# ignacio-rocco/detectorch

Measured on AMD Instinct MI355X. Metric: images/sec Mask R-CNN R-50-FPN 1333x800 (region-proposal hot path), higher is better.
Workload: dtype f32

## Files before the change

### detectorch_amd/csrc/roi_align_tile.hip

```cpp

#include <type_traits>

#include "roi_align_common.h"

namespace dtc {

constexpr int kTileMaxK = 32;
constexpr int kTileRoiBytes = 48, kTileGroupBytes = 32;
constexpr int kTileHdrBytes = kTileMaxK * (kTileRoiBytes + kTileGroupBytes) + 16;
template <int NT> struct TileShape;
template <> struct TileShape<256> { static constexpr int kUnits = 8, kWaves = 3, kLdsKB = 52, kWaves16 = 4, kLds16KB = 38; };

struct TileRoi {
  int lvl, b, x0, x1, y0, y1, r, valid;
  float sh, sw, bin_h, bin_w;
};
static_assert(sizeof(TileRoi) == kTileRoiBytes, "TileRoi layout");
struct TileGroup { int first, count, kind, x0, x1, y0, y1, pad; };
enum { kGrpPool = 0, kGrpZero = 1, kGrpAbsent = 2, kGrpGather = 3 };

__device__ __forceinline__ __amdgpu_buffer_rsrc_t make_srd(const void* base) {
  return __builtin_amdgcn_make_buffer_rsrc(const_cast<void*>(base), 0, 0xffffffff, 0x00020000);
}
template <typename TIn> struct Piece4;
template <> struct Piece4<float> {
  typedef float4 Raw;
  static __device__ __forceinline__ Raw raw(__amdgpu_buffer_rsrc_t r, uint32_t voff, uint32_t soff) {
    const u32x4 v = __builtin_amdgcn_raw_buffer_load_b128(r, voff, soff, 0);
    return make_float4(__uint_as_float(v.x), __uint_as_float(v.y), __uint_as_float(v.z), __uint_as_float(v.w));
  }
};
template <> struct Piece4<__half> {
  typedef u32x2 Raw;
  static __device__ __forceinline__ Raw raw(__amdgpu_buffer_rsrc_t r, uint32_t voff, uint32_t soff) { return __builtin_amdgcn_raw_buffer_load_b64(r, voff, soff, 0); }
};
template <> struct Piece4<bf16_t> {
  typedef u32x2 Raw;
  static __device__ __forceinline__ Raw raw(__amdgpu_buffer_rsrc_t r, uint32_t voff, uint32_t soff) { return __builtin_amdgcn_raw_buffer_load_b64(r, voff, soff, 0); }
};

template <typename TIn> struct TileLds { typedef float T; static constexpr int kSlot = 16, kShift = 4; };
template <> struct TileLds<__half> { typedef uint16_t T; static constexpr int kSlot = 8, kShift = 3; };
template <> struct TileLds<bf16_t> { typedef uint16_t T; static constexpr int kSlot = 8, kShift = 3; };

template <typename TIn, int NT> struct TileBounds { static constexpr int kWaves = TileShape<NT>::kWaves; };
template <int NT> struct TileBounds<__half, NT> { static constexpr int kWaves = TileShape<NT>::kWaves16; };
template <int NT> struct TileBounds<bf16_t, NT> { static constexpr int kWaves = TileShape<NT>::kWaves16; };

__device__ __forceinline__ int tile_phys(int px) { return px + (px >> 3); }

struct TileItem {
  int a[2][2][4];
  float yl[2], yh[2], xl[2], xh[2];
  bool on;
};

enum { kStageScalar = 0, kStageVec = 1, kStageVecUnaligned = 2 };

struct TileGeom {
  int first, count;
  int y0, x0a, ngx, npos;
  int plane;
  int nq_pass;
  int mode;
};

template <typename TIn, typename TOut, int NT, bool FUSED>
__device__ __forceinline__ void tile_passes(const RoiAlignParams& p, const dtc_feat_level& L, const TIn* fbase, int c0, int nc,
                                            int bins, float* slab, typename TileLds<TIn>::T* win, const TileRoi* troi, const TileGeom& g,
                                            const TileItem& it, int rl, int bin) {
  constexpr int NW = NT / 64;
  constexpr int U = TileShape<NT>::kUnits;
  typedef typename TileLds<TIn>::T TL;
  constexpr bool L16 = sizeof(TL) == 2;
  constexpr int SB = TileLds<TIn>::kSlot;
  const int tid = threadIdx.x, lane = tid & 63, wv = tid >> 6, pl = lane & 15, cl = (lane >> 4) & 3;
  const int npos = g.npos, ngx = g.ngx, plane = g.plane, nq_pass = g.nq_pass;
  const int nchunk = (npos + 15) >> 4;
  const int KC = ceil_div(nchunk, NW);
  const float rinv = 1.0f / (float)ngx;
  const int nq_tot = ceil_div(nc, 4);
  const bool vec = g.mode != kStageScalar;
  uint32_t uoff[U];
  int ulds[U];
  const int nu = KC * nq_pass;
  if (vec) {
    const int sh32 = (int)L.stride_h, sc32 = (int)L.stride_c;
    int q = 0, i = 0;
#pragma unroll
    for (int u = 0; u < U; u++) {
      const bool dup = u >= nu;
      const int pos = min((wv + (dup ? 0 : i) * NW) * 16 + pl, npos - 1);
      const int row = (int)(((float)pos + 0.5f) * rinv);
      const int gx = pos - row * ngx;
      const int qq = dup ? 0 : q;
      int col = g.x0a + 4 * gx, sft = 0;
      if (g.mode == kStageVecUnaligned) { sft = max(0, col + 3 - (L.width - 1)); col -= sft; }
      uoff[u] = ((uint32_t)((g.y0 + row) * sh32 + col + (4 * qq + cl) * sc32) * (uint32_t)sizeof(TIn)) | ((uint32_t)sft << 30);
      ulds[u] = qq * plane * 4 + ((4 * pos + (pos >> 1)) << 2) + cl;
      if (++i == KC) { i = 0; q++; }
    }
  }
  const __amdgpu_buffer_rsrc_t srd = make_srd(fbase);
  const uint32_t pass_bytes = (uint32_t)(L.stride_c * (int64_t)sizeof(TIn));
  typename Piece4<TIn>::Raw v[U];
  auto issue = [&](int cs) {
    const uint32_t soff = (uint32_t)cs * pass_bytes;
    if (g.mode == kStageVec) {
#pragma unroll
      for (int u = 0; u < U; u++) v[u] = Piece4<TIn>::raw(srd, uoff[u], soff);
    } else {
#pragma unroll
      for (int u = 0; u < U; u++) v[u] = Piece4<TIn>::raw(srd, uoff[u] & 0x3fffffffu, soff);
    }
  };
  auto commit_as = [&](auto shifted_tag) {
    constexpr bool SHIFTED = decltype(shifted_tag)::value;
    if constexpr (SHIFTED) asm volatile("" ::: "memory");
#pragma unroll
    for (int u = 0; u < U; u++) {
      if constexpr (L16) {
        uint32_t w0 = v[u].x & 0xffffu, w1 = v[u].x >> 16, w2 = v[u].y & 0xffffu, w3 = v[u].y >> 16;
        if constexpr (SHIFTED) {
          const uint32_t sft = uoff[u] >> 30;
          w0 = sft == 0 ? w0 : sft == 1 ? w1 : sft == 2 ? w2 : w3;
          w1 = sft == 0 ? w1 : sft == 1 ? w2 : w3;
          w2 = sft == 0 ? w2 : w3;
        }
        TL* d = win + ulds[u];
        d[0] = (TL)w0; d[4] = (TL)w1; d[8] = (TL)w2; d[12] = (TL)w3;
      } else {
        float4 w = v[u];
        if constexpr (SHIFTED) {
          const uint32_t sft = uoff[u] >> 30;
          w.x = sft == 0 ? w.x : sft == 1 ? w.y : sft == 2 ? w.z : w.w;
          w.y = sft == 0 ? w.y : sft == 1 ? w.z : w.w;
          w.z = sft == 0 ? w.z : w.w;
        }
        TL* d = win + ulds[u];
        d[0] = w.x; d[4] = w.y; d[8] = w.z; d[12] = w.w;
      }
    }
  };
  auto commit = [&]() {
    if (g.mode == kStageVecUnaligned) commit_as(std::true_type{}); else commit_as(std::false_type{});
  };
  auto lds_val = [&](const TIn& x) -> TL {
    if constexpr (L16) return *reinterpret_cast<const uint16_t*>(&x); else return to_f32<TIn>(x);
  };
  auto stage_scalar = [&](int cs) {
#pragma unroll 1
    for (int q = 0; q < nq_pass; q++) {
      const int cq = cs + 4 * q;
      if (cq >= nc) break;
      const int cle = min(cl, nc - 1 - cq);
      const TIn* base = fbase + (int64_t)(cq + cle) * L.stride_c;
#pragma unroll 1
      for (int t = wv; t < nchunk; t += NW) {
        const int pos = min(t * 16 + pl, npos - 1);
        const int row = (int)(((float)pos + 0.5f) * rinv);
        const int gx = pos - row * ngx;
        const int rem = L.width - 1 - (g.x0a + 4 * gx);
        const TIn* s = base + (int64_t)(g.y0 + row) * L.stride_h + (int64_t)(g.x0a + 4 * gx) * L.stride_w;
        TL* d = win + q * plane * 4 + ((4 * pos + (pos >> 1)) << 2) + cl;
        d[0] = lds_val(s[0]);
        d[4] = lds_val(s[(int64_t)min(1, rem) * L.stride_w]);
        d[8] = lds_val(s[(int64_t)min(2, rem) * L.stride_w]);
        d[12] = lds_val(s[(int64_t)min(3, rem) * L.stride_w]);
      }
    }
  };
  const bool quad_ok = ((p.channels | c0) & 3) == 0;
  auto store_slab = [&](int cs, int nq) {
    const int nch = min(4 * nq, nc - cs);
    TOut* out = reinterpret_cast<TOut*>(p.out);
    if (quad_ok && nch == 4 * nq) {
      const int n4 = nq * bins, total = g.count * n4;
      const float r4 = 1.0f / (float)n4;
      const int cs_off = cs * bins;
      for (int idx = tid; idx < total; idx += NT) {
        const int k = (int)(((float)idx + 0.5f) * r4);
        const int e = idx - __mul24(k, n4);
        const float4 val = reinterpret_cast<const float4*>(slab)[idx];
        const uint64_t ob = *reinterpret_cast<const uint64_t*>(&troi[g.first + k].x0);
        store4<TOut>(out + (ob + (uint64_t)(uint32_t)(cs_off + 4 * e)), val);
      }
    } else {
      const int per = nch * bins, total = g.count * per;
      for (int idx = tid; idx < total; idx += NT) {
        const int k = idx / per, e = idx - k * per;
        out[((size_t)troi[g.first + k].r * p.channels + c0 + cs) * bins + e] = from_f32<TOut>(slab[k * 4 * nq * bins + e]);
      }
    }
  };

  if (vec) issue(0);
  int cs_prev = 0, nq_prev = 0;
#pragma unroll 1
  for (int qs = 0; qs < nq_tot; qs += nq_pass) {
    const int cs = 4 * qs;
    const int nq_cur = min(nq_pass, nq_tot - qs);
    if (vec) commit(); else stage_scalar(cs);
    if (nq_prev) store_slab(cs_prev, nq_prev);
    __syncthreads();
    if (vec && qs + nq_pass < nq_tot) issue(cs + 4 * nq_pass);
    if (it.on) {
      float* so = slab + rl * (4 * nq_cur * bins) + bin;
#pragma unroll 1
      for (int q = 0; q < nq_cur; q++) {
        const char* wq = reinterpret_cast<const char*>(win) + uni(q * plane * SB);
        f32x2 a01 = {0.f, 0.f}, a23 = {0.f, 0.f};
#pragma unroll
        for (int iy = 0; iy < 2; iy++) {
          if constexpr (L16 && FUSED) {
            u32x2 t[2][4];
#pragma unroll
            for (int ix = 0; ix < 2; ix++)
#pragma unroll
              for (int k = 0; k < 4; k++)
                t[ix][k] = *reinterpret_cast<const u32x2*>(__builtin_assume_aligned(wq + it.a[iy][ix][k], 8));
#pragma unroll
            for (int ix = 0; ix < 2; ix++) {
              const float w1 = it.yh[iy] * it.xh[ix], w2 = it.yh[iy] * it.xl[ix];
              const float w3 = it.yl[iy] * it.xh[ix], w4 = it.yl[iy] * it.xl[ix];
              fma_pair16<TIn>(a01, t[ix][0].x, w1); fma_pair16<TIn>(a23, t[ix][0].y, w1);
              fma_pair16<TIn>(a01, t[ix][1].x, w2); fma_pair16<TIn>(a23, t[ix][1].y, w2);
              fma_pair16<TIn>(a01, t[ix][2].x, w3); fma_pair16<TIn>(a23, t[ix][2].y, w3);
              fma_pair16<TIn>(a01, t[ix][3].x, w4); fma_pair16<TIn>(a23, t[ix][3].y, w4);
            }
          } else if constexpr (L16) {
            u32x2 t[2][4];
#pragma unroll
            for (int ix = 0; ix < 2; ix++)
#pragma unroll
              for (int k = 0; k < 4; k++)
                t[ix][k] = *reinterpret_cast<const u32x2*>(__builtin_assume_aligned(wq + it.a[iy][ix][k], 8));
#pragma unroll
            for (int ix = 0; ix < 2; ix++) {
              const float w1 = it.yh[iy] * it.xh[ix], w2 = it.yh[iy] * it.xl[ix];
              const float w3 = it.yl[iy] * it.xh[ix], w4 = it.yl[iy] * it.xl[ix];
              f32x2 s01 = mul_pair16<TIn>(t[ix][0].x, w1) + mul_pair16<TIn>(t[ix][1].x, w2);
              s01 = s01 + mul_pair16<TIn>(t[ix][2].x, w3);
              s01 = s01 + mul_pair16<TIn>(t[ix][3].x, w4);
              f32x2 s23 = mul_pair16<TIn>(t[ix][0].y, w1) + mul_pair16<TIn>(t[ix][1].y, w2);
              s23 = s23 + mul_pair16<TIn>(t[ix][2].y, w3);
              s23 = s23 + mul_pair16<TIn>(t[ix][3].y, w4);
              a01 = a01 + s01; a23 = a23 + s23;
            }
          } else {
            f32x4 t[2][4];
#pragma unroll
            for (int ix = 0; ix < 2; ix++)
#pragma unroll
              for (int k = 0; k < 4; k++)
                t[ix][k] = *reinterpret_cast<const f32x4*>(__builtin_assume_aligned(wq + it.a[iy][ix][k], 16));
#pragma unroll
            for (int ix = 0; ix < 2; ix++) {
              const float w1 = it.yh[iy] * it.xh[ix], w2 = it.yh[iy] * it.xl[ix];
              const float w3 = it.yl[iy] * it.xh[ix], w4 = it.yl[iy] * it.xl[ix];
              a01 += w1 * t[ix][0].lo + w2 * t[ix][1].lo + w3 * t[ix][2].lo + w4 * t[ix][3].lo;
              a23 += w1 * t[ix][0].hi + w2 * t[ix][1].hi + w3 * t[ix][2].hi + w4 * t[ix][3].hi;
            }
          }
          __builtin_amdgcn_sched_barrier(0);
        }
        float* o = so + uni(4 * q * bins);
        const float a0 = a01.x, a1 = a01.y, a2 = a23.x, a3 = a23.y;
        o[0] = a0 * 0.25f; o[bins] = a1 * 0.25f; o[2 * bins] = a2 * 0.25f; o[3 * bins] = a3 * 0.25f;
      }
    }
    __syncthreads();
    cs_prev = cs; nq_prev = nq_cur;
  }
  if (nq_prev) store_slab(cs_prev, nq_prev);
}

__device__ __forceinline__ int tile_work_item(int b, int n, int reverse) {
  if (n < 2 * kXcds || (reverse & 2)) return (reverse & 1) ? n - 1 - b : b;
  const int x = b % kXcds, j = b / kXcds;
  const int q = n / kXcds, r = n - q * kXcds;
  const int start = x * q + min(x, r), qx = q + (x < r ? 1 : 0);
  return start + ((reverse & 1) ? qx - 1 - j : j);
}

template <typename TIn, typename TOut, int NT, bool FUSED>
__global__ __launch_bounds__(NT, (TileBounds<TIn, NT>::kWaves)) void roi_align_fwd_tile(RoiAlignParams p, int kgroup, int lds_bytes, int nq_cap, int merge_pct, int reverse) {
  extern __shared__ __attribute__((aligned(16))) unsigned char smem[];
  TileRoi* troi = reinterpret_cast<TileRoi*>(smem);
  TileGroup* tgrp = reinterpret_cast<TileGroup*>(smem + kTileMaxK * kTileRoiBytes);
  int* ngp = reinterpret_cast<int*>(smem + kTileMaxK * (kTileRoiBytes + kTileGroupBytes));
  const int slab_bytes = kgroup * p.pooled_h * p.pooled_w * 16 * nq_cap;
  float* slab = reinterpret_cast<float*>(smem + kTileHdrBytes);
  typedef typename TileLds<TIn>::T TL;
  constexpr int SB = TileLds<TIn>::kSlot;
  TL* win = reinterpret_cast<TL*>(smem + kTileHdrBytes + slab_bytes);
  const int win_bytes = lds_bytes - kTileHdrBytes - slab_bytes;
  constexpr int NW = NT / 64;
  constexpr int kMaxPos = TileShape<NT>::kUnits * NW * 16;
  const int tid = threadIdx.x;
  const int nct = ceil_div(p.channels, p.ch_block);
  const int wi = tile_work_item(blockIdx.x, gridDim.x, reverse);
  int grp = wi / nct;
  int c0 = (wi - grp * nct) * p.ch_block;
  {
    const int ngrp = (int)gridDim.x / nct;
    if ((reverse & 4) && ngrp % kXcds == 0 && ngrp >= 2 * kXcds) {
      const int x = blockIdx.x % kXcds, j = blockIdx.x / kXcds, ngx = ngrp / kXcds;
      const int cbi = j / ngx, gl = j - cbi * ngx;
      grp = x * ngx + ((reverse & 1) ? ngx - 1 - gl : gl);
      c0 = cbi * p.ch_block;
    }
  }
  const int nc = min(p.ch_block, p.channels - c0);
  const int bins = p.pooled_h * p.pooled_w;
  const int K = kgroup;

  if (tid < 64) {
    TileRoi t;
    t.lvl = -1; t.b = 0; t.x0 = t.x1 = t.y0 = t.y1 = 0; t.r = 0; t.valid = 0; t.sh = t.sw = 0.f; t.bin_h = t.bin_w = 1.f;
    const int ri = grp * K + tid;
    if (tid < K && ri < p.n_rois) {
      const RoiHead hd = load_roi_head(p, ri);
      t.valid = 1; t.r = hd.r; t.b = hd.b; t.sh = hd.sh; t.sw = hd.sw; t.bin_h = hd.bin_h; t.bin_w = hd.bin_w;
      if (hd.lvl >= 0 && hd.lvl < p.n_levels) {
        t.lvl = hd.lvl;
        const int H = p.lv[hd.lvl].height, W = p.lv[hd.lvl].width;
        t.y0 = make_axis(hd.sh, hd.bin_h, 0, 0, 2, H).lo;
        t.y1 = make_axis(hd.sh, hd.bin_h, p.pooled_h - 1, 1, 2, H).hi;
        t.x0 = make_axis(hd.sw, hd.bin_w, 0, 0, 2, W).lo;
        t.x1 = make_axis(hd.sw, hd.bin_w, p.pooled_w - 1, 1, 2, W).hi;
      }
    }
    if (tid < K) {
      troi[tid] = t;
      *reinterpret_cast<uint64_t*>(&troi[tid].x0) = ((uint64_t)(uint32_t)t.r * (uint64_t)p.channels + (uint64_t)c0) * (uint64_t)(p.pooled_h * p.pooled_w);
    }
    auto bc = [](int v, int k) { return __builtin_amdgcn_readlane(v, k); };
    int ng = 0, k = 0;
    while (k < K) {
      const int ks = uni(k);
      const int a_lvl = bc(t.lvl, ks), a_b = bc(t.b, ks), a_valid = bc(t.valid, ks);
      const int a_x0 = bc(t.x0, ks), a_x1 = bc(t.x1, ks), a_y0 = bc(t.y0, ks), a_y1 = bc(t.y1, ks);
      TileGroup g;
      g.first = k; g.count = 1; g.x0 = a_x0; g.x1 = a_x1; g.y0 = a_y0; g.y1 = a_y1; g.pad = 0;
      if (!a_valid) g.kind = kGrpAbsent;
      else if (a_lvl < 0) g.kind = kGrpZero;
      else {
        const int ngx0 = (a_x1 >> 2) - (a_x0 >> 2) + 1, th0 = a_y1 - a_y0 + 1, npos0 = th0 * ngx0;
        if (npos0 > kMaxPos || (4 * npos0 + (npos0 >> 1) + 1) * SB > win_bytes || bins > NT) {
          g.kind = kGrpGather;
        } else {
          g.kind = kGrpPool;
          long long sum_px = (long long)th0 * (a_x1 - a_x0 + 1);
          while (k + g.count < K && (g.count + 1) * bins <= NT) {
            const int js = uni(k + g.count);
            const int n_lvl = bc(t.lvl, js), n_b = bc(t.b, js), n_valid = bc(t.valid, js);
            if (!n_valid || n_lvl != a_lvl || n_b != a_b) break;
            const int n_x0 = bc(t.x0, js), n_x1 = bc(t.x1, js), n_y0 = bc(t.y0, js), n_y1 = bc(t.y1, js);
            const int ux0 = min(g.x0, n_x0), ux1 = max(g.x1, n_x1), uy0 = min(g.y0, n_y0), uy1 = max(g.y1, n_y1);
            const int ungx = (ux1 >> 2) - (ux0 >> 2) + 1, uth = uy1 - uy0 + 1, unpos = uth * ungx;
            if (unpos > kMaxPos || (4 * unpos + (unpos >> 1) + 1) * SB > win_bytes) break;
            const long long n_px = (long long)(n_y1 - n_y0 + 1) * (n_x1 - n_x0 + 1);
            const long long u_px = (long long)uth * (ux1 - ux0 + 1);
            if (u_px * 100 > (sum_px + n_px) * merge_pct) break;
            g.x0 = ux0; g.x1 = ux1; g.y0 = uy0; g.y1 = uy1; g.count++;
            sum_px += n_px;
          }
        }
      }
      if (tid == 0) tgrp[ng] = g;
      ng++;
      k += g.count;
    }
    if (tid == 0) *ngp = ng;
  }
  __syncthreads();

  const int ngroups = uni(*ngp);
  for (int gi = 0; gi < ngroups; gi++) {
    const int first = uni(tgrp[gi].first), count = uni(tgrp[gi].count), kind = uni(tgrp[gi].kind);
    if (kind == kGrpAbsent) continue;
    if (kind == kGrpZero) {
      TOut* oz = reinterpret_cast<TOut*>(p.out) + ((size_t)uni(troi[first].r) * p.channels + c0) * bins;
      zero_outputs<TOut, NT>(oz, nc * bins, tid);
      continue;
    }
    const int lvl = uni(troi[first].lvl), b = uni(troi[first].b);
    const dtc_feat_level L = p.lv[lvl];
    const TIn* fbase = reinterpret_cast<const TIn*>(L.data) + (int64_t)b * L.stride_n + (int64_t)c0 * L.stride_c;
    if (kind == kGrpGather) {
      const RoiHead hd = load_roi_head(p, grp * K + first);
      TOut* og = reinterpret_cast<TOut*>(p.out) + ((size_t)hd.r * p.channels + c0) * bins;
      for (int o = tid; o < nc * bins; o += NT) {
        const int c = o / bins, bin = o - c * bins;
        const int ph = bin / p.pooled_w, pw = bin - ph * p.pooled_w;
        const TIn* d = fbase + (int64_t)c * L.stride_c;
        float acc = 0.f;
        for (int iy = 0; iy < 2; iy++) {
          const AxisEntry y = make_axis(hd.sh, hd.bin_h, ph, iy, 2, L.height);
          const int64_t ylo = (int64_t)y.lo * L.stride_h, yhi = (int64_t)y.hi * L.stride_h;
          for (int ix = 0; ix < 2; ix++) {
            const AxisEntry x = make_axis(hd.sw, hd.bin_w, pw, ix, 2, L.width);
            const int64_t xlo = (int64_t)x.lo * L.stride_w, xhi = (int64_t)x.hi * L.stride_w;
            const float w1 = y.h * x.h, w2 = y.h * x.l, w3 = y.l * x.h, w4 = y.l * x.l;
            acc += w1 * to_f32<TIn>(d[ylo + xlo]) + w2 * to_f32<TIn>(d[ylo + xhi]) + w3 * to_f32<TIn>(d[yhi + xlo]) +
                   w4 * to_f32<TIn>(d[yhi + xhi]);
          }
        }
        og[o] = from_f32<TOut>(acc * 0.25f);
      }
      continue;
    }
    const int gx0 = uni(tgrp[gi].x0), gx1 = uni(tgrp[gi].x1), gy0 = uni(tgrp[gi].y0), gy1 = uni(tgrp[gi].y1);
    TileGeom g;
    g.first = first; g.count = count;
    g.y0 = gy0; g.x0a = gx0 & ~3;
    g.ngx = (gx1 >> 2) - (gx0 >> 2) + 1;
    const int tw = 4 * g.ngx, th = gy1 - gy0 + 1;
    g.npos = th * g.ngx;
    g.plane = 4 * g.npos + (g.npos >> 1) + 1;
    const int esz = (int)sizeof(TIn);
    const bool lin = L.stride_w == 1 && ((nc | c0) & 3) == 0 && L.stride_h > 0 && L.stride_c > 0 &&
                     L.stride_h * L.height + L.stride_c * 4 * TileShape<NT>::kUnits < (1ll << 26);
    const bool al16 = ((L.width | L.stride_h | L.stride_c | L.stride_n) & 3) == 0 &&
                      (reinterpret_cast<uintptr_t>(L.data) & (4 * sizeof(TIn) - 1)) == 0;
    const bool al4 = L.width >= 4 && (((L.width | L.stride_h | L.stride_c | L.stride_n) * esz) & 3) == 0 &&
                     (reinterpret_cast<uintptr_t>(L.data) & 3) == 0;
    g.mode = !lin ? kStageScalar : al16 ? kStageVec : al4 ? kStageVecUnaligned : kStageScalar;
    const int KC = ceil_div((g.npos + 15) >> 4, NW);
    g.nq_pass = max(1, min(min(win_bytes / (g.plane * SB), TileShape<NT>::kUnits / KC), min(ceil_div(nc, 4), nq_cap)));
    while (ceil_div(nc, 4) % g.nq_pass) g.nq_pass--;
    const int n_it = count * bins;
    TileItem it;
    it.on = tid < n_it;
    const int itx = it.on ? tid : 0;
    const int rl = itx / bins, bin = itx - rl * bins;
    const int ph = bin / p.pooled_w, pw = bin - ph * p.pooled_w;
    const TileRoi hd = troi[first + rl];
    int ylo[2], yhi[2], xlo[2], xhi[2];
#pragma unroll
    for (int i = 0; i < 2; i++) {
      const AxisEntry ey = make_axis(hd.sh, hd.bin_h, ph, i, 2, L.height);
      const AxisEntry ex = make_axis(hd.sw, hd.bin_w, pw, i, 2, L.width);
      it.yl[i] = ey.l; it.yh[i] = ey.h; it.xl[i] = ex.l; it.xh[i] = ex.h;
      ylo[i] = (ey.lo - gy0) * tw; yhi[i] = (ey.hi - gy0) * tw;
      xlo[i] = ex.lo - g.x0a; xhi[i] = ex.hi - g.x0a;
    }
#pragma unroll
    for (int iy = 0; iy < 2; iy++)
#pragma unroll
      for (int ix = 0; ix < 2; ix++) {
        constexpr int SS = TileLds<TIn>::kShift;
        int t0 = tile_phys(ylo[iy] + xlo[ix]) << SS, t1 = tile_phys(ylo[iy] + xhi[ix]) << SS;
        int t2 = tile_phys(yhi[iy] + xlo[ix]) << SS, t3 = tile_phys(yhi[iy] + xhi[ix]) << SS;
        asm volatile("" : "+v"(t0), "+v"(t1), "+v"(t2), "+v"(t3));
        it.a[iy][ix][0] = t0; it.a[iy][ix][1] = t1; it.a[iy][ix][2] = t2; it.a[iy][ix][3] = t3;
      }
    tile_passes<TIn, TOut, NT, FUSED>(p, L, fbase, c0, nc, bins, slab, win, troi, g, it, rl, bin);
  }
}

constexpr int kTileThreads = 256;
constexpr int kTileMergePct = 250;
constexpr int kTileNqCap = 4;
constexpr int kTileReverse = 1;

template <typename TIn, typename TOut, int NT, bool FUSED>
static int launch_tile_nt(RoiAlignParams p, hipStream_t stream) {
  const RoiAlignKnobs& cfg = roi_align_knobs();
  const int bins = p.pooled_h * p.pooled_w;
  int K = NT / bins;
  K = K < 1 ? 1 : (K > kTileMaxK ? kTileMaxK : K);
  if (K * bins > NT) K = NT / bins;
  if (K < 1) return DTC_EUNSUPPORTED;
  const int lds_b = (sizeof(TIn) == 2 ? (cfg.tile_lds16_kb ? cfg.tile_lds16_kb : TileShape<NT>::kLds16KB) : TileShape<NT>::kLdsKB) * 1024;
  if (raise_lds_once<roi_align_fwd_tile<TIn, TOut, NT, FUSED>>() != DTC_OK) return DTC_ELAUNCH;
  const int nq_cap = kTileNqCap;
  if (kTileHdrBytes + K * bins * 16 * nq_cap + 20 * 1024 > lds_b) return DTC_EUNSUPPORTED;
  const int ngrp = ceil_div(p.n_rois, K);
  int cb = cfg.tile_ch_block ? cfg.tile_ch_block : ((long long)ngrp * ceil_div(p.channels, 128) >= 6144 ? 128 : 64);
  while (!cfg.tile_ch_block && cb > 32 && (long long)ngrp * ceil_div(p.channels, cb) < 2048) cb >>= 1;
  p.ch_block = cb;
  const int nct = ceil_div(p.channels, p.ch_block);
  hipLaunchKernelGGL((roi_align_fwd_tile<TIn, TOut, NT, FUSED>), dim3((unsigned)ngrp * nct), dim3(NT), lds_b, stream, p, K, lds_b, nq_cap, kTileMergePct, (kTileReverse ? 1 : 0) | (p.xcd_remap ? 0 : 2) | (cfg.tile_cb_major ? 4 : 0));
  DTC_CHECK_LAUNCH();
  return DTC_OK;
}

template <typename TIn, typename TOut>
static int launch_tile_t(const RoiAlignParams& p, hipStream_t stream) {
  if constexpr (sizeof(TIn) == 2) { if (!roi_align_get_exact()) return launch_tile_nt<TIn, TOut, kTileThreads, true>(p, stream); }
  return launch_tile_nt<TIn, TOut, kTileThreads, false>(p, stream);
}

bool roi_align_tile_supported(const RoiAlignParams& p, int in_dtype, int out_dtype) {
  if (p.sampling_ratio != 2) return false;
  if (p.pooled_h * p.pooled_w > kTileThreads) return false;
  return io_pair_supported(in_dtype, out_dtype);
}

int launch_roi_align_tile(const RoiAlignParams& p, int in_dtype, int out_dtype, hipStream_t stream) {
  if (p.n_rois == 0) return DTC_OK;
  return dispatch_io_pair(in_dtype, out_dtype, [&](auto tin, auto tout) {
    return launch_tile_t<tag_type<decltype(tin)>, tag_type<decltype(tout)>>(p, stream);
  });
}

}
```

Baseline: 14500.

## Add per-row coverage table so merged ROI groups skip uncovered feature pixels

When several ROIs are merged into one bounding window, the kernel now builds a per-row coverage table in the spare ROI-header LDS that records each row's covered column span. Staging loads clamp columns to that span and redirect uncovered rows to a covered source row, so redundant loads hit the same cache lines instead of fetching unused pixels. This adds a COV template variant, extra setup loops during group formation, and register and LDS use. It relies on the unused header space being large enough, and the window stays the same size.

```diff
diff --git a/detectorch_amd/csrc/roi_align_tile.hip b/detectorch_amd/csrc/roi_align_tile.hip
--- a/detectorch_amd/csrc/roi_align_tile.hip
+++ b/detectorch_amd/csrc/roi_align_tile.hip
@@ -16,8 +16,11 @@
   float sh, sw, bin_h, bin_w;
 };
 static_assert(sizeof(TileRoi) == kTileRoiBytes, "TileRoi layout");
-struct TileGroup { int first, count, kind, x0, x1, y0, y1, pad; };
+struct TileGroup { int first, count, kind, x0, x1, y0, y1, cov; };
 enum { kGrpPool = 0, kGrpZero = 1, kGrpAbsent = 2, kGrpGather = 3 };
+
+constexpr int kTileCovRows = 64;
+constexpr int kTileCovBytes = kTileCovRows * 4;
 
 __device__ __forceinline__ __amdgpu_buffer_rsrc_t make_srd(const void* base) {
   return __builtin_amdgcn_make_buffer_rsrc(const_cast<void*>(base), 0, 0xffffffff, 0x00020000);
@@ -63,9 +66,10 @@
   int plane;
   int nq_pass;
   int mode;
+  const uint32_t* cov;
 };
 
-template <typename TIn, typename TOut, int NT, bool FUSED>
+template <typename TIn, typename TOut, int NT, bool FUSED, bool COV>
 __device__ __forceinline__ void tile_passes(const RoiAlignParams& p, const dtc_feat_level& L, const TIn* fbase, int c0, int nc,
                                             int bins, float* slab, typename TileLds<TIn>::T* win, const TileRoi* troi, const TileGeom& g,
                                             const TileItem& it, int rl, int bin) {
@@ -91,9 +95,14 @@
     for (int u = 0; u < U; u++) {
       const bool dup = u >= nu;
       const int pos = min((wv + (dup ? 0 : i) * NW) * 16 + pl, npos - 1);
-      const int row = (int)(((float)pos + 0.5f) * rinv);
-      const int gx = pos - row * ngx;
+      int row = (int)(((float)pos + 0.5f) * rinv);
+      int gx = pos - row * ngx;
       const int qq = dup ? 0 : q;
+      if (COV && g.cov) {
+        const uint32_t rec = g.cov[row];
+        gx = min(max(gx, (int)(rec & 0xffu)), (int)((rec >> 8) & 0xffu));
+        row = (int)(rec >> 16);
+      }
       int col = g.x0a + 4 * gx, sft = 0;
       if (g.mode == kStageVecUnaligned) { sft = max(0, col + 3 - (L.width - 1)); col -= sft; }
       uoff[u] = ((uint32_t)((g.y0 + row) * sh32 + col + (4 * qq + cl) * sc32) * (uint32_t)sizeof(TIn)) | ((uint32_t)sft << 30);
@@ -283,12 +292,14 @@
   return start + ((reverse & 1) ? qx - 1 - j : j);
 }
 
-template <typename TIn, typename TOut, int NT, bool FUSED>
+template <typename TIn, typename TOut, int NT, bool FUSED, bool COV>
 __global__ __launch_bounds__(NT, (TileBounds<TIn, NT>::kWaves)) void roi_align_fwd_tile(RoiAlignParams p, int kgroup, int lds_bytes, int nq_cap, int merge_pct, int reverse) {
   extern __shared__ __attribute__((aligned(16))) unsigned char smem[];
   TileRoi* troi = reinterpret_cast<TileRoi*>(smem);
   TileGroup* tgrp = reinterpret_cast<TileGroup*>(smem + kTileMaxK * kTileRoiBytes);
   int* ngp = reinterpret_cast<int*>(smem + kTileMaxK * (kTileRoiBytes + kTileGroupBytes));
+  uint32_t* cov_tab = reinterpret_cast<uint32_t*>(smem + kgroup * kTileRoiBytes);
+  const int cov_tables = (kTileMaxK - kgroup) * kTileRoiBytes / kTileCovBytes;
   const int slab_bytes = kgroup * p.pooled_h * p.pooled_w * 16 * nq_cap;
   float* slab = reinterpret_cast<float*>(smem + kTileHdrBytes);
   typedef typename TileLds<TIn>::T TL;
@@ -336,13 +347,13 @@
       *reinterpret_cast<uint64_t*>(&troi[tid].x0) = ((uint64_t)(uint32_t)t.r * (uint64_t)p.channels + (uint64_t)c0) * (uint64_t)(p.pooled_h * p.pooled_w);
     }
     auto bc = [](int v, int k) { return __builtin_amdgcn_readlane(v, k); };
-    int ng = 0, k = 0;
+    int ng = 0, k = 0, ncov = 0;
     while (k < K) {
       const int ks = uni(k);
       const int a_lvl = bc(t.lvl, ks), a_b = bc(t.b, ks), a_valid = bc(t.valid, ks);
       const int a_x0 = bc(t.x0, ks), a_x1 = bc(t.x1, ks), a_y0 = bc(t.y0, ks), a_y1 = bc(t.y1, ks);
       TileGroup g;
-      g.first = k; g.count = 1; g.x0 = a_x0; g.x1 = a_x1; g.y0 = a_y0; g.y1 = a_y1; g.pad = 0;
+      g.first = k; g.count = 1; g.x0 = a_x0; g.x1 = a_x1; g.y0 = a_y0; g.y1 = a_y1; g.cov = 0;
       if (!a_valid) g.kind = kGrpAbsent;
       else if (a_lvl < 0) g.kind = kGrpZero;
       else {
@@ -366,6 +377,20 @@
             g.x0 = ux0; g.x1 = ux1; g.y0 = uy0; g.y1 = uy1; g.count++;
             sum_px += n_px;
           }
+          const int th = g.y1 - g.y0 + 1, px0 = g.x0 >> 2;
+          if (COV && g.count > 1 && th <= kTileCovRows && (g.x1 >> 2) - px0 < 256 && ncov < cov_tables) {
+            const int y = g.y0 + tid;
+            int lo = 255, hi = 0;
+            for (int m = 0; m < g.count; m++) {
+              const int ms = uni(k + m);
+              const int m_x0 = bc(t.x0, ms), m_x1 = bc(t.x1, ms), m_y0 = bc(t.y0, ms), m_y1 = bc(t.y1, ms);
+              if (y >= m_y0 && y <= m_y1) { lo = min(lo, (m_x0 >> 2) - px0); hi = max(hi, (m_x1 >> 2) - px0); }
+            }
+            int src = tid;
+            if (lo > hi) { lo = hi = (a_x0 >> 2) - px0; src = a_y0 - g.y0; }
+            if (tid < th) cov_tab[ncov * kTileCovRows + tid] = (uint32_t)lo | ((uint32_t)hi << 8) | ((uint32_t)src << 16);
+            g.cov = ++ncov;
+          }
         }
       }
       if (tid == 0) tgrp[ng] = g;
@@ -427,6 +452,8 @@
     const bool al4 = L.width >= 4 && (((L.width | L.stride_h | L.stride_c | L.stride_n) * esz) & 3) == 0 &&
                      (reinterpret_cast<uintptr_t>(L.data) & 3) == 0;
     g.mode = !lin ? kStageScalar : al16 ? kStageVec : al4 ? kStageVecUnaligned : kStageScalar;
+    const int cov = uni(tgrp[gi].cov);
+    g.cov = COV && cov ? cov_tab + (cov - 1) * kTileCovRows : nullptr;
     const int KC = ceil_div((g.npos + 15) >> 4, NW);
     g.nq_pass = max(1, min(min(win_bytes / (g.plane * SB), TileShape<NT>::kUnits / KC), min(ceil_div(nc, 4), nq_cap)));
     while (ceil_div(nc, 4) % g.nq_pass) g.nq_pass--;
@@ -456,7 +483,7 @@
         asm volatile("" : "+v"(t0), "+v"(t1), "+v"(t2), "+v"(t3));
         it.a[iy][ix][0] = t0; it.a[iy][ix][1] = t1; it.a[iy][ix][2] = t2; it.a[iy][ix][3] = t3;
       }
-    tile_passes<TIn, TOut, NT, FUSED>(p, L, fbase, c0, nc, bins, slab, win, troi, g, it, rl, bin);
+    tile_passes<TIn, TOut, NT, FUSED, COV>(p, L, fbase, c0, nc, bins, slab, win, troi, g, it, rl, bin);
   }
 }
 
@@ -474,7 +501,8 @@
   if (K * bins > NT) K = NT / bins;
   if (K < 1) return DTC_EUNSUPPORTED;
   const int lds_b = (sizeof(TIn) == 2 ? (cfg.tile_lds16_kb ? cfg.tile_lds16_kb : TileShape<NT>::kLds16KB) : TileShape<NT>::kLdsKB) * 1024;
-  if (raise_lds_once<roi_align_fwd_tile<TIn, TOut, NT, FUSED>>() != DTC_OK) return DTC_ELAUNCH;
+  const bool cov = K > 1;
+  if ((cov ? raise_lds_once<roi_align_fwd_tile<TIn, TOut, NT, FUSED, true>>() : raise_lds_once<roi_align_fwd_tile<TIn, TOut, NT, FUSED, false>>()) != DTC_OK) return DTC_ELAUNCH;
   const int nq_cap = kTileNqCap;
   if (kTileHdrBytes + K * bins * 16 * nq_cap + 20 * 1024 > lds_b) return DTC_EUNSUPPORTED;
   const int ngrp = ceil_div(p.n_rois, K);
@@ -482,7 +510,9 @@
   while (!cfg.tile_ch_block && cb > 32 && (long long)ngrp * ceil_div(p.channels, cb) < 2048) cb >>= 1;
   p.ch_block = cb;
   const int nct = ceil_div(p.channels, p.ch_block);
-  hipLaunchKernelGGL((roi_align_fwd_tile<TIn, TOut, NT, FUSED>), dim3((unsigned)ngrp * nct), dim3(NT), lds_b, stream, p, K, lds_b, nq_cap, kTileMergePct, (kTileReverse ? 1 : 0) | (p.xcd_remap ? 0 : 2) | (cfg.tile_cb_major ? 4 : 0));
+  const int order = (kTileReverse ? 1 : 0) | (p.xcd_remap ? 0 : 2) | (cfg.tile_cb_major ? 4 : 0);
+  if (cov) hipLaunchKernelGGL((roi_align_fwd_tile<TIn, TOut, NT, FUSED, true>), dim3((unsigned)ngrp * nct), dim3(NT), lds_b, stream, p, K, lds_b, nq_cap, kTileMergePct, order);
+  else hipLaunchKernelGGL((roi_align_fwd_tile<TIn, TOut, NT, FUSED, false>), dim3((unsigned)ngrp * nct), dim3(NT), lds_b, stream, p, K, lds_b, nq_cap, kTileMergePct, order);
   DTC_CHECK_LAUNCH();
   return DTC_OK;
 }
```

Result: faster. 14750, median of 6 (+1.7%).
